# InterDigitalInc/VersatileFilmGrain

Hardware: AMD Instinct MI355X
Metric: Mpixels/s (Y+UV) + achieved HBM GB/s vs roofline, 4320p 10-bit 4:2:0 (higher is better)
Workload: dtype u16

## Files before the change

include/vfgs_hip.h:

```cpp
#ifndef VFGS_HIP_H
#define VFGS_HIP_H

#include <stdint.h>

#ifdef __cplusplus
extern "C" {
#endif

#define VFGS_HIP_MAX_PATTERNS 8


void vfgs_set_luma_pattern(int index, signed char* P);
void vfgs_set_chroma_pattern(int index, signed char* P);
void vfgs_set_scale_lut(int c, unsigned char lut[]);
void vfgs_set_pattern_lut(int c, unsigned char lut[]);
void vfgs_set_seed(unsigned int seed);
void vfgs_set_scale_shift(int shift);
void vfgs_set_depth(int depth);
void vfgs_set_legal_range(int legal);
void vfgs_set_chroma_subsampling(int subx, int suby);
void vfgs_add_grain_line(void* Y, void* U, void* V, int y, int width);


void vfgs_hip_line_lookahead(int enable);
// ... 87 lines not shown
int vfgs_hip_overlap_end(void* stream);

int vfgs_hip_init_devices(const int* devices, int n);

int vfgs_hip_supports_depth(int depth);

int vfgs_hip_dev_build(void);

int vfgs_hip_add_grain_frames_host(void* const* Y, void* const* U, void* const* V, unsigned nframes, unsigned width,
                                   unsigned height, unsigned stride, unsigned cstride);
void* vfgs_hip_host_alloc(uint64_t bytes);
void vfgs_hip_host_free(void* p);

int vfgs_hip_device_info(int* cu_count, int* lds_bytes_per_cu, int* clock_khz, char* name, int name_len);

typedef struct vfgs_hip_launch_info {
	int depth, csubx, csuby;
	int out8;
	int one_y, one_c;
	int in_place;
	int nframes;
	int workgroups_per_frame;
	int frames_per_front;
	int rows_per_wave[2];
	int positions_per_row[2];
	int parts_per_row;
	int persistent_luma_workgroups;
	int waves_per_workgroup;
	int lds_bytes_per_workgroup;
	unsigned long long launches;
	char kernel[96];
	int listed;
	int internal;
} vfgs_hip_launch_info;
int vfgs_hip_last_launch_info(vfgs_hip_launch_info* out);

#ifdef __cplusplus
}
#endif

#endif
```

versatilefilmgrain_amd/csrc/vfgs_fw_kernel.hip:

```cpp
#include <hip/hip_runtime.h>

#include "vfgs_fw_layout.h"
#include "vfgs_layout.h"

namespace vfgs {
namespace {

__device__ inline int noise_index(const uint32_t* w, int n)
{
	const uint64_t two = ((uint64_t)w[(n >> 5) + 1] << 32) | w[n >> 5];
	return (int)((two >> (n & 31)) & 2047u);
}

__device__ inline int clip127(int v) { return v > 127 ? 127 : (v < -127 ? -127 : v); }

__device__ inline void put_sample(const FwLaunch& L, const vfgs_hip_pattern_job& jb, int y, int x, int v)
{
	if (!jb.chroma)
		L.bank[(size_t)jb.index * 4096 + y * 64 + x] = (int8_t)v;
	else if (L.csubx == 2 && L.csuby == 2)
		L.bank[(size_t)(kSlots + jb.index) * 4096 + y * 64 + x] = (int8_t)v;
	else
		L.chroma_raw[jb.index * 1024 + y * 32 + x] = (int8_t)v;
}
// ... 231 lines not shown
	ImageLayout L;
	int one_y, one_c, slot_y, slot_cb, slot_cr;
	int pk16;
};

__global__ __launch_bounds__(256) void fw_patch_tables(const PatchArgs p)
{
	const int o = blockIdx.x * 256 + threadIdx.x;
	const ImageLayout& L = p.L;
	if (o < 64 * 64)
	{
		const int r = o >> 6, x = o & 63;
		uint8_t* dst = p.img + L.y_off + L.y_bank;
		if (p.one_y)
		{
			if (p.slot_y < kSlots && (p.mask_luma >> p.slot_y & 1))
			{
				const int v = p.bank[(size_t)p.slot_y * 4096 + o];
				if (p.pk16)
				{
					*(int16_t*)(dst + r * L.y_rs + 2 * x) = (int16_t)v;
					*(int16_t*)(dst + L.y_neg + r * L.y_rs + 2 * x) = (int16_t)-v;
				}
				else
				{
					dst[r * L.y_rs + x] = (uint8_t)v;
					dst[L.y_neg + r * L.y_rs + x] = (uint8_t)-v;
				}
			}
		}
		else
			for (int k = 0; k < kSlots; k++)
				if (p.mask_luma >> k & 1)
					dst[r * L.y_rs + x * kSlots + k] = (uint8_t)p.bank[(size_t)k * 4096 + o];
	}
	else if (o - 4096 < L.cw * L.ch)
	{
		const int q = o - 4096;
		const int r = q / L.cw, x = q % L.cw;
		if (p.one_c)
		{
			for (int c = 0; c < 2; c++)
			{
				const int k = c ? p.slot_cr : p.slot_cb;
				if (k < kSlots && (p.mask_chroma >> k & 1))
				{
					const int v = p.bank[(size_t)(kSlots + k) * 4096 + r * 64 + x];
					if (p.pk16)
					{
						*(int16_t*)(p.img + L.c_off[c] + L.c_bank + r * L.c_rs + 2 * x) = (int16_t)v;
						*(int16_t*)(p.img + L.c_off[c] + L.c_bank + L.c_neg + r * L.c_rs + 2 * x) = (int16_t)-v;
					}
					else
					{
						p.img[L.c_off[c] + L.c_bank + r * L.c_rs + x] = (uint8_t)v;
						p.img[L.c_off[c] + L.c_bank + L.c_neg + r * L.c_rs + x] = (uint8_t)-v;
					}
				}
			}
		}
		else
			for (int k = 0; k < kSlots; k++)
				if (p.mask_chroma >> k & 1)
					for (int c = 0; c < 2; c++)
						p.img[L.c_off[c] + L.c_bank + r * L.c_rs + x * kSlots + k] = (uint8_t)p.bank[(size_t)(kSlots + k) * 4096 + r * 64 + x];
	}
}

}

hipError_t launch_fw_generate(const FwLaunch& L, hipStream_t stream)
{
	bool ff = false, ar = false, chroma = false;
	for (int i = 0; i < L.njobs; i++)
	{
		(L.job[i].kind ? ar : ff) = true;
		chroma = chroma || L.job[i].chroma;
	}
	if (ff) hipLaunchKernelGGL(fw_ff_kernel, dim3(L.njobs), dim3(1024), 0, stream, L);
	if (ar) hipLaunchKernelGGL(fw_ar_kernel, dim3(L.njobs), dim3(256), 0, stream, L);
	if (chroma && !(L.csubx == 2 && L.csuby == 2))
		hipLaunchKernelGGL(fw_commit_chroma, dim3(L.njobs), dim3(256), 0, stream, L);
	return hipGetLastError();
}

hipError_t launch_fw_patch(uint8_t* img, const int8_t* bank, uint32_t mask_luma, uint32_t mask_chroma, int csubx, int csuby,
                           bool one_y, bool one_c, int slot_y, int slot_cb, int slot_cr, bool depth8, hipStream_t stream)
{
	PatchArgs p{};
	p.img = img; p.bank = bank; p.mask_luma = mask_luma; p.mask_chroma = mask_chroma;
	p.L = image_layout(csubx, csuby, one_y, one_c, depth8);
	p.pk16 = depth8 && kPk16;
	p.one_y = one_y; p.one_c = one_c; p.slot_y = slot_y; p.slot_cb = slot_cb; p.slot_cr = slot_cr;
	const int n = 4096 + p.L.cw * p.L.ch;
	hipLaunchKernelGGL(fw_patch_tables, dim3((n + 255) / 256), dim3(256), 0, stream, p);
	return hipGetLastError();
}

// ... 2 lines not shown
```

versatilefilmgrain_amd/csrc/vfgs_host.cpp:

```cpp
#include <hip/hip_runtime.h>

#include <sys/mman.h>
#include <unistd.h>

#include <algorithm>
#include <chrono>
#if defined(__SSE2__)
#include <emmintrin.h>
#endif
#include <cstdarg>
#include <cstdio>
#include <cstdlib>
#include <cstring>
#include <mutex>
#include <string>
#include <thread>
#include <vector>

#include "../../include/vfgs_hip.h"
#include "../../include/vfgs_hip_fw.h"
#include "vfgs_fw_layout.h"
#include "vfgs_layout.h"

namespace vfgs {
// ... 1006 lines not shown

int uniform_slot(const uint8_t (&plut)[256])
{
	const int k = plut[0] >> 4;
	for (int i = 1; i < 256; i++)
		if ((plut[i] >> 4) != k) return -1;
	return k;
}

void build_tables(const State& s, uint8_t* img, const vfgs::ImageLayout& L, bool one_y, bool one_c, const int (&slot)[3])
{
	memset(img, 0, L.bytes);
	const bool pk16 = s.bs == 0 && vfgs::kPk16;
	uint8_t* yb = img + L.y_off + L.y_bank;
	for (int r = 0; r < 64; r++)
		for (int x = 0; x < 64; x++)
		{
			if (one_y)
			{
				const int v = slot[0] < vfgs::kSlots ? s.bank[0][slot[0]][r][x] : 0;
				if (pk16)
				{
					const int16_t p = (int16_t)v, n = (int16_t)-v;
					memcpy(yb + r * L.y_rs + 2 * x, &p, 2);
					memcpy(yb + L.y_neg + r * L.y_rs + 2 * x, &n, 2);
				}
				else
				{
					yb[r * L.y_rs + x] = (uint8_t)v;
					yb[L.y_neg + r * L.y_rs + x] = (uint8_t)-v;
				}
			}
			else
				for (int k = 0; k < vfgs::kSlots; k++) yb[r * L.y_rs + x * vfgs::kSlots + k] = (uint8_t)s.bank[0][k][r][x];
		}
	for (int c = 0; c < 2; c++)
	{
		uint8_t* cb = img + L.c_off[c] + L.c_bank;
		for (int r = 0; r < L.ch; r++)
			for (int x = 0; x < L.cw; x++)
			{
				if (one_c)
				{
					const int v = slot[1 + c] < vfgs::kSlots ? s.bank[1][slot[1 + c]][r][x] : 0;
					if (pk16)
					{
						const int16_t p = (int16_t)v, n = (int16_t)-v;
						memcpy(cb + r * L.c_rs + 2 * x, &p, 2);
						memcpy(cb + L.c_neg + r * L.c_rs + 2 * x, &n, 2);
					}
					else
					{
						cb[r * L.c_rs + x] = (uint8_t)v;
						cb[L.c_neg + r * L.c_rs + x] = (uint8_t)-v;
					}
				}
				else
					for (int k = 0; k < vfgs::kSlots; k++) cb[r * L.c_rs + x * vfgs::kSlots + k] = (uint8_t)s.bank[1][k][r][x];
			}
	}
	for (int c = 0; c < 3; c++)
	{
		uint32_t* lut = (uint32_t*)(c == 0 ? img + L.y_off : img + L.c_off[c - 1] + L.c_lut[c - 1]);
		if (pk16 && (c == 0 ? one_y : one_c))
		{
			memcpy(lut, s.slut[c], 256);
			continue;
		}
		for (int i = 0; i < 256; i++)
		{
			const int sl = s.plut[c][i] >> 4;
			const uint32_t sel = sl < vfgs::kSlots ? (uint32_t)sl : 0x0cu;
			const int sc = s.slut[c][i] << (16 - s.scale_shift);
			lut[i] = (sel << 24) | ((uint32_t)sc & 0xffffffu);
			if (!(c == 0 ? one_y : one_c)) lut[256 + i] = (sel << 24) | ((uint32_t)(-sc) & 0xffffffu);
		}
	}
}

void digest_pluts(State& s)
{
	if (s.plut_seen) return;
	s.plut_bad_c = -1;
	for (int c = 0; c < 3; c++)
	{
		s.plut_slot[c] = uniform_slot(s.plut[c]);
		for (int i = 0; i < 256 && s.plut_bad_c < 0; i++)
			if ((s.plut[c][i] >> 4) > vfgs::kSlots) { s.plut_bad_c = c; s.plut_bad_i = i; }
	}
	s.plut_seen = true;
}
// ... 290 lines not shown
	}
	else
	{
		if (int e = upload_stream(s, lo, hi, stream)) return e;
		HIP_TRY(s.lfsr.use(stream));
		a.stream = s.lfsr.dev();
		a.stream_bytes = (uint32_t)(s.lfsr.dev_words() * 4);
		a.cur_bit0 = (uint32_t)(first_cur - s.lfsr.base_bit());
		a.up_bit0 = (uint32_t)(first_up - s.lfsr.base_bit());
		a.frame_bit_step = (uint32_t)frame_step;
	}

	const long per_frame = (long)a.pd[0].wgs + 2L * a.pd[1].wgs;
	if (per_frame > 0x3fffffffL || nframes > 65535) return fail(14, "launch too large");
	if (per_frame == 0) { if (seeds) seeded_done(); return 0; }
	bool persist = false;
	long grid = per_frame;
	if (VFGS_PERSIST_MIN_TASKS > 0 && s.bs != 0 && !wide && !s.img_one_y && a.pd[0].wgs > 0 &&
	    (size_t)vfgs::kWavesPerWG * a.pd[0].rw_rpw * a.pd[0].rowbytes <= ((size_t)VFGS_PERSIST_MAX_WG_KB << 10))
	{
		const long tasks = (long)a.pd[0].wgs * nframes, slots = (long)s.cu_count * 4;
		const long k = (tasks + slots - 1) / slots;
		if (k >= VFGS_PERSIST_MIN_TASKS)
		{
			const long P = (tasks + k - 1) / k;
			persist = true;
			a.persist_wgs = (int)P;
			a.persist_step_f = (int)(P / a.pd[0].wgs);
			a.persist_step_r = (int)(P % a.pd[0].wgs);
			grid = P + 2L * a.pd[1].wgs * nframes;
			if (grid > 0x7fffffffL) return fail(14, "launch too large");
		}
	}
#ifdef VFGS_NO_FRONTS
	a.lfronts = 0;
#else
	const bool in_region = g_states[0].ov.active && (stream == g_states[0].ov.s[0] || stream == g_states[0].ov.s[1]);
	a.lfronts = (!persist && nframes >= 2 && !in_region && 2 * (yext + 2 * cext) >= (64u << 20)) ? 1 : 0;
#endif
	if (mix)
	{
		if (!(s.img_one_y && s.img_one_c) || persist) return fail(19, "internal: the table image is not the form the chroma mix was admitted for");
		a.mix_kernel = 1;
		a.mix_lw = (int)width;
		for (int c = 0; c < 2; c++)
		{
			a.mix[c][0] = g_mix[c][0]; a.mix[c][1] = g_mix[c][1];
			a.mix[c][2] = g_mix[c][2] * (1 << s.bs);
			a.mix[c][3] = g_mix[c][3];
		}
		const uint64_t dext = dg.out8 ? (uint64_t)part_h * dg.stride : yext, dfp = dg.out8 ? dg.ypitch : ypitch;
		auto meet = [](uintptr_t p, uint64_t pn, uintptr_t q, uint64_t qn) { return p < q + qn && q < p + pn; };
		bool shared = false;
		if (!list)
			shared = meet((uintptr_t)sY, (uint64_t)(nframes - 1) * ypitch + yext, (uintptr_t)dY, (uint64_t)(nframes - 1) * dfp + dext);
		else
			for (unsigned i = 0; i < nframes && !shared; i++)
				for (unsigned j = 0; j < nframes && !shared; j++)
					shared = meet((uintptr_t)list->src[0][i], yext, (uintptr_t)list->dst[0][j], dext);
		if (shared)
		{
			a.mix_planes = 1;
			HIP_TRY(vfgs::launch_grain(a, list, 8 + s.bs, s.csubx, s.csuby, dg.out8, true, true, wide, false, (int)grid, stream));
			a.mix_planes = 2;
		}
	}
	HIP_TRY(vfgs::launch_grain(a, list, 8 + s.bs, s.csubx, s.csuby, dg.out8, s.img_one_y, s.img_one_c, wide, persist, (int)grid, stream));
	if (seeds) seeded_done();
	if (stripes && s.stripes.prepare_next(s.lfsr) != hipSuccess) (void)hipGetLastError();
	if (&s == &g_states[0])
	{
		vfgs_hip_launch_info& li = g_last_launch;
		const unsigned long long n = li.launches + 1;
		li = vfgs_hip_launch_info{};
		li.launches = n;
		li.depth = 8 + s.bs; li.csubx = s.csubx; li.csuby = s.csuby;
		li.out8 = dg.out8; li.one_y = s.img_one_y; li.one_c = s.img_one_c;
		li.in_place = (sY == dY && sU == dU && sV == dV);
		li.listed = a.listed;
		li.internal = g_internal_launch ? 1 : 0;
		li.nframes = (int)nframes;
		li.workgroups_per_frame = (int)per_frame;
		li.frames_per_front = 1 << a.lfronts;
		for (int pt = 0; pt < 2; pt++)
		{
			li.rows_per_wave[pt] = a.pd[pt].rw_rpw;
			li.positions_per_row[pt] = a.pd[pt].rw_segs;
		}
		li.parts_per_row = (int)nparts;
		li.persistent_luma_workgroups = persist ? a.persist_wgs : 0;
		li.waves_per_workgroup = vfgs::kWavesPerWG;
		const vfgs::ImageLayout L = vfgs::layout_of(s.csubx, s.csuby, s.img_one_y, s.img_one_c, s.bs == 0);
		li.lds_bytes_per_workgroup = vfgs::lds_allocation(s.bs != 0, s.img_one_y, s.img_one_c, wide, L.lds_bytes + vfgs::kParamBytes);
		vfgs::describe_launch(li.kernel, sizeof li.kernel, 8 + s.bs, s.csubx, s.csuby, dg.out8, s.img_one_y, s.img_one_c, wide, persist);
		if (mix)
		{
			li.lds_bytes_per_workgroup = vfgs::mix_lds_allocation(L.lds_bytes + vfgs::kParamBytes);
			snprintf(li.kernel, sizeof li.kernel, "grain_mix_kernel<%d,%d,%d,%s,%s>", 8 + s.bs, s.csubx, s.csuby, dg.out8 ? "true" : "false", wide ? "true" : "false");
			if (a.mix_planes) li.launches++;
		}
		g_last_launch_valid = true;
	}
	return 0;
}

int run_host(void* Y, void* U, void* V, unsigned y, unsigned width, unsigned height, unsigned stride, unsigned cstride, unsigned py, unsigned ph)
{
	State& s = S();
	if (int e = ensure_init(-1)) return e;
	if (height == 0) return 0;
	const unsigned sz = s.bs ? 2 : 1;
	const unsigned nblk = (width + 15) / 16;
	if (ph == 0)
	{
		if (int e = check_luts(s)) return e;
		advance_seeds(s, y, height, nblk, y);
		return 0;
	}
	const unsigned crow0 = py / s.csuby;
	const unsigned crows = (py + ph - 1) / s.csuby - crow0 + 1;
	const unsigned rows[3] = {ph, crows, crows};
	const unsigned rowlen[3] = {nblk * 16 * sz, nblk * 16 / s.csubx * sz, nblk * 16 / s.csubx * sz};
// ... 1374 lines not shown
```

versatilefilmgrain_amd/csrc/vfgs_kernel.hip:

```cpp
#include <hip/hip_runtime.h>
#include <stdint.h>
#include <stdio.h>

#include <type_traits>

#include "vfgs_layout.h"

namespace vfgs {

typedef uint32_t u32x4 __attribute__((ext_vector_type(4)));
typedef uint32_t u32x2 __attribute__((ext_vector_type(2)));
typedef uint32_t u32x3 __attribute__((ext_vector_type(3)));
typedef short s16x2 __attribute__((ext_vector_type(2)));
typedef unsigned short u16x2 __attribute__((ext_vector_type(2)));


__device__ __forceinline__ int pick_slot(uint32_t hi, uint32_t lo, uint32_t lut_entry)
{
	return (int)__builtin_amdgcn_perm(hi, lo, lut_entry) >> 24;
}

__device__ __forceinline__ int mad_i24(int x, uint32_t y, int c)
{
	int r;
// ... 60 lines not shown
constexpr uint32_t kOOB = 0x80000000u;

__device__ __forceinline__ __amdgpu_buffer_rsrc_t make_rsrc(const uint8_t* base, uint32_t bytes)
{
	return __builtin_amdgcn_make_buffer_rsrc((void*)base, 0, bytes, 0x00020000);
}

template <int NS, int BW>
struct LaneMap {
	static constexpr bool PAIR = (NS == 8 && BW == 16);
	static constexpr int SHIFT = PAIR ? 8 : BW / 2;
	static constexpr int NR = PAIR ? 1 : NS / BW + 1;
	static constexpr int NQ = NS / 4;
	static constexpr int NE = NR - 1;
	static constexpr int BPL = PAIR ? 1 : NS / BW;
	__device__ static constexpr int run(int q) { return PAIR ? 0 : (4 * q + BW - SHIFT) / BW; }
	__device__ static constexpr int col(int q) { return PAIR ? 4 * q : (4 * q + BW - SHIFT) % BW; }
	__device__ static constexpr int edge_quad(int e) { return PAIR ? 0 : ((e + 1) * BW - (BW - SHIFT)) / 4 - 1; }
};

template <int NR>
struct RunParam {
	uint32_t pa[NR];
};

template <int SUBX, int SUBY, int RS, int SB>
__device__ __forceinline__ uint32_t block_param(uint32_t v, uint32_t bank_off, int sx, int sy, int sb, bool* neg)
{
	const uint32_t fx = (v >> sx) & 0x3ff;
	const uint32_t fy = __builtin_amdgcn_alignbit(v, v, sy) & 0x3ff;
	const uint32_t ox = (__umul24(fx, 13u) >> 10) * (4 / SUBX);
	const uint32_t oy = (__umul24(fy, 12u) >> 10) * (4 / SUBY);
	*neg = (v >> sb) & 1;
	return __umul24(oy, (uint32_t)RS) + ox * SB + bank_off;
}

template <int DEPTH, int BW, bool OVERLAP, bool ONE, bool ALIGN2, int NEG, bool MIX = false>
__device__ __forceinline__ void grain_unit(const uint8_t* lds, uint32_t (&w)[4],
                                            const RunParam<LaneMap<DEPTH == 8 ? 16 : 8, BW>::NR>& rp,
                                            const RunParam<LaneMap<DEPTH == 8 ? 16 : 8, BW>::NR>& up,
                                            const uint32_t lutb, const uint32_t rowoff, const uint32_t uprowoff, const int wcur, const int wup,
                                            const bool (&edge_on)[LaneMap<DEPTH == 8 ? 16 : 8, BW>::PAIR ? 1 : LaneMap<DEPTH == 8 ? 16 : 8, BW>::NE],
                                            const bool first, const uint32_t lo2, const uint32_t hi2, const int pkshift, const uint32_t (&ix)[4])
{
	constexpr int NS = DEPTH == 8 ? 16 : 8;
	using M = LaneMap<NS, BW>;
	constexpr int NR = M::NR, NQ = M::NQ;
	auto index_dword = [&](int d) { return MIX ? ix[d] : w[d]; };
	constexpr bool PK = DEPTH == 8 && ONE && kPk16;
	static_assert(!(PK && M::PAIR), "lane pairs are 10-bit lanes");
	int sg[NR];
	uint32_t ad[NR], k2s[NR];
#pragma unroll
	for (int r = 0; r < NR; r++)
	{
		sg[r] = (int)rp.pa[r] >> 31;
		ad[r] = (rp.pa[r] & 0xffffu) + rowoff - ((ONE && OVERLAP) ? ((uint32_t)sg[r] & (uint32_t)NEG) : 0u);
		k2s[r] = ONE ? 0u : (OVERLAP ? lutb : (((uint32_t)sg[r] & 0x04000400u) | lutb));
	}
	if constexpr (PK && !OVERLAP)
	{
		const uint32_t rnd = 1u << (pkshift - 1);
		const uint32_t rpk = rnd * 0x10001u, shpk = (uint32_t)pkshift * 0x10001u;
		const uint8_t* lut = lds + (lutb & 0xffffu);
		uint32_t S[NS / 2], Pp[NS / 2], G[NS / 2];
#pragma unroll
		for (int q = 0; q < NQ; q++)
// ... 326 lines not shown
{
	constexpr int NS = DEPTH == 8 ? 16 : 8;
	constexpr int SZ = DEPTH > 8 ? 2 : 1;
	constexpr int SB = ONE ? ((DEPTH == 8 && kPk16) ? 2 : 1) : kSlots;
	using M = LaneMap<NS, BW>;
	constexpr int NR = M::NR;
	constexpr int RPB = 16 / SUBY;
	constexpr int NEF = M::PAIR ? 1 : M::NE;
	constexpr int K = M::SHIFT * SZ / 4;
	constexpr int DW = OUT8 ? 2 : 4;
	constexpr int KD = OUT8 ? K / 2 : K;
	static_assert(!OUT8 || (DEPTH > 8 && K % 2 == 0), "the narrowed destination exists for 16-bit containers");
	constexpr int LDA = VFGS_LDAUX_ALIGNED, STA = VFGS_STAUX_ALIGNED;
	constexpr int LPB = M::PAIR ? 1 : M::BPL;
	constexpr int BPS = M::PAIR ? 32 : 64 * M::BPL;
	constexpr int NU = MIX ? 2 : ((DEPTH > 8 && ONE && NARROW != 0) ? VFGS_RING_NARROW10 : ring_depth<DEPTH, ONE>());
	constexpr int GPP = kTileBlocks / (NU * BPS);
	static_assert(GPP * NU * BPS == kTileBlocks, "a part is a whole number of groups");
	constexpr uint32_t PT_CUR = IMG_BYTES, PT_UP = IMG_BYTES + kParamTableBytes;
	static_assert(IMG_BYTES % 16 == 0, "table image in whole 16-byte units");
	static_assert(!(PERSIST && (WIDE || NARROW != 0)), "persistent workgroups walk ordinary rows");
	static_assert(!MIX || (ONE && NARROW == 0 && !PERSIST), "the mix exists for one-pattern chroma walked row by row");
	const int pt = comp ? 1 : 0;
	auto uni = [](int v) { return __builtin_amdgcn_readfirstlane(v); };

	auto task = [&](const int f, const int r, const bool first_task) {
	const int split = r & (pd.rw_splits - 1);
	const int kbr = uni(r >> pd.rw_lsplits);
	const int Rabs = (a.y0 >> 4) + kbr;
	const int row_first = (a.y0 + SUBY - 1) / SUBY;
	const int prow0 = a.y0 / SUBY;
	const int alo = max(row_first, Rabs * RPB), ahi = min(row_first + pd.nrows, (Rabs + 1) * RPB);
	const int rpw = pd.rw_rpw;
#if VFGS_RW_CONSEC
	const int RSTR = 1;
	const int base = uni(Rabs * RPB + split * (kWavesPerWG * rpw) + wave * rpw);
	int k0 = max(0, alo - base), k1 = min(rpw, max(0, ahi - base));
#else
	constexpr int RSTR = kWavesPerWG;
	const int base = uni(Rabs * RPB + split * (kWavesPerWG * rpw) + wave);
	int k0 = (max(0, alo - base) + kWavesPerWG - 1) / kWavesPerWG, k1 = min(rpw, (max(0, ahi - base) + kWavesPerWG - 1) / kWavesPerWG);
#endif
	if (kbr >= a.nbrows || k1 < k0) k1 = k0;
	k0 = uni(k0); k1 = uni(k1);
	const bool wg_up = (Rabs > 0) && (split == 0);

	const int last = a.nblk - 1;
	const uint32_t cur_bit = a.cur_bit0 + (uint32_t)f * a.frame_bit_step + (uint32_t)(kbr * a.nblk);
	const uint32_t up_bit = (kbr > 0) ? cur_bit - (uint32_t)a.nblk : a.up_bit0 + (uint32_t)f * a.frame_bit_step;

	constexpr int STEP = kWavesPerWG * 64 * 16;
	constexpr int NIT = (IMG_BYTES + STEP - 1) / STEP;
	u32x4 tmp[NIT];
	if (!PERSIST || first_task)
	{
		const __amdgpu_buffer_rsrc_t irs = make_rsrc(a.tables + img_off, IMG_BYTES);
#pragma unroll
		for (int it = 0; it < NIT; it++)
			tmp[it] = __builtin_amdgcn_raw_buffer_load_b128(irs, min((uint32_t)(threadIdx.x * 16 + it * STEP), (uint32_t)(IMG_BYTES - 16)), 0, 0);
	}
	constexpr int NPE = (kParamEntries + kWavesPerWG * 64 - 1) / (kWavesPerWG * 64);
	const __amdgpu_buffer_rsrc_t strs = make_rsrc((const uint8_t*)a.stream, a.stream_bytes);
	const __amdgpu_buffer_rsrc_t strs_up = make_rsrc((const uint8_t*)a.stream, wg_up ? a.stream_bytes : 0);
	auto param_loads = [&](const int B0, u32x2 (&wc)[NPE], u32x2 (&wu)[NPE]) {
#pragma unroll
		for (int i = 0; i < NPE; i++)
		{
			const int e = (int)threadIdx.x + i * kWavesPerWG * 64;
			const uint32_t blk = (uint32_t)min(max(B0 + e - 1, 0), last);
			const bool need = e < a.nblk - B0 + 4 && e < kParamEntries;
			wc[i] = __builtin_amdgcn_raw_buffer_load_b64(strs, need ? ((cur_bit + blk) >> 5) * 4 : kOOB, 0, 0);
			wu[i] = __builtin_amdgcn_raw_buffer_load_b64(strs_up, need ? ((up_bit + blk) >> 5) * 4 : kOOB, 0, 0);
		}
	};
	const int fsx = comp == 0 ? 0 : (comp == 1 ? 10 : 20);
	const int fsy = comp == 0 ? 14 : (comp == 1 ? 24 : 4);
	const int fsb = comp == 0 ? 31 : (comp == 1 ? 2 : 15);
	auto param_table = [&](const int B0, const u32x2 (&wc)[NPE], const u32x2 (&wu)[NPE]) {
#pragma unroll
		for (int i = 0; i < NPE; i++)
		{
			if (i > 0 && i * kWavesPerWG * 64 >= a.nblk - B0 + 4) break;
			const int e = (int)threadIdx.x + i * kWavesPerWG * 64;
			const uint32_t blk = (uint32_t)min(max(B0 + e - 1, 0), last);
			bool neg;
			const uint32_t vc = __builtin_amdgcn_alignbit(wc[i].y, wc[i].x, (cur_bit + blk) & 31);
			const uint32_t pc = (block_param<SUBX, SUBY, RS, SB>(vc, bank_off, fsx, fsy, fsb, &neg) + ((ONE && neg) ? (uint32_t)NEG : 0u)) | (neg ? 0x80000000u : 0u);
			const uint32_t vu = __builtin_amdgcn_alignbit(wu[i].y, wu[i].x, (up_bit + blk) & 31);
			const uint32_t pu = block_param<SUBX, SUBY, RS, SB>(vu, bank_off, fsx, fsy, fsb, &neg) | (neg ? 0x80000000u : 0u);
			if (e < kParamEntries)
			{
				*(uint32_t*)(lds + PT_CUR + e * 4) = pc;
// ... 29 lines not shown
			lw[u][4 * i] = t.x; lw[u][4 * i + 1] = t.y; lw[u][4 * i + 2] = t.z; lw[u][4 * i + 3] = t.w;
		}
	};
	if constexpr (NARROW == 0)
	{
		const __amdgpu_buffer_rsrc_t rs0 = make_rsrc(sbase + (k0 < k1 ? row_off(k0) : 0u), k0 < k1 ? left(0) : 0u);
#pragma unroll
		for (int u = 0; u < NU; u++) load_seg<LDA>(rs0, lane16 + u * UB, 0, w[u]);
		if constexpr (MIX)
		{
#pragma unroll
			for (int u = 0; u < NU; u++)
			{
				const uint32_t o = (uint32_t)u * (UB * LQ);
				const bool on = k0 < k1 && o < pl.rowbytes;
				load_luma(make_rsrc(lbase + (on ? lrow_off(k0) + o : 0u), on ? min(pl.rowbytes - o, UB * LQ) : 0u), u);
			}
		}
	}
	else
	{
#pragma unroll
		for (int u = 0; u < NU; u++)
		{
			const int k = k0 + u / NARROW;
			const __amdgpu_buffer_rsrc_t rs0 = make_rsrc(sbase + (k < k1 ? row_off(k) : 0u), k < k1 ? pd.rowbytes : 0u);
			load_seg<LDA>(rs0, lane16 + (u % NARROW) * UB, 0, w[u]);
		}
	}
	if (!PERSIST || first_task)
	{
#pragma unroll
		for (int it = 0; it < NIT; it++)
			*(u32x4*)(lds + min((uint32_t)(threadIdx.x * 16 + it * STEP), (uint32_t)(IMG_BYTES - 16))) = tmp[it];
	}
	else
		__syncthreads();

	param_table(0, wc0, wu0);
	__syncthreads();
	const int nparts = WIDE ? (a.nblk + kTileBlocks - 1) / kTileBlocks : 1;
	static_assert(!(WIDE && NARROW != 0), "rows walked in parts are not narrow");
	if (k0 >= k1 && nparts == 1)
		return;

	const uint32_t lutb = lut_off * 0x10001u;
	const uint32_t lo2 = a.lo2[pt], hi2 = a.hi2[pt];
	const bool first = M::PAIR && (lane & 1);
	const uint32_t pairoff = M::PAIR ? (first ? 0u : 8u * SB) : 0u;
	const uint32_t idx0 = (M::PAIR ? (uint32_t)(lane + 1) >> 1 : (uint32_t)lane * LPB) * 4;
	const int cl = M::PAIR ? lane - 1 - (lane & 1) : lane * LPB - 1;
	constexpr int SSTEP = M::PAIR ? 64 : BPS;
	auto lane_up = [](uint32_t old, uint32_t v) { return (uint32_t)__builtin_amdgcn_update_dpp((int)old, (int)v, 0x138, 0xf, 0xf, false); };
	auto lane_down = [](uint32_t old, uint32_t v) { return (uint32_t)__builtin_amdgcn_update_dpp((int)old, (int)v, 0x130, 0xf, 0xf, false); };
	auto rot_up = [](uint32_t v) { return (uint32_t)__builtin_amdgcn_mov_dpp((int)v, 0x13c, 0xf, 0xf, false); };
	auto rot_down = [](uint32_t v) { return (uint32_t)__builtin_amdgcn_mov_dpp((int)v, 0x134, 0xf, 0xf, false); };
	auto results = [](const uint32_t (&t)[4], uint32_t (&o)[DW]) {
		if constexpr (OUT8)
		{
			uint32_t n[4];
#pragma unroll
			for (int d = 0; d < 4; d++) n[d] = ((t[d] + (0x00010001u << (DEPTH - 9))) >> (DEPTH - 8)) & 0x00ff00ffu;
			o[0] = __builtin_amdgcn_perm(n[1], n[0], 0x06040200);
			o[1] = __builtin_amdgcn_perm(n[3], n[2], 0x06040200);
		}
		else
		{
// ... 7 lines not shown
	const int mixc = comp == 2 ? 1 : 0;
	const int mix_lm = MIX ? a.mix[mixc][0] : 0, mix_cm = MIX ? a.mix[mixc][1] : 0, mix_off = MIX ? a.mix[mixc][2] : 0;
	const bool mix_on = MIX && a.mix[mixc][3] != 0;
	uint32_t outp[DW] = {};
	uint32_t tp[KD > 0 ? KD : 1] = {};
	__amdgpu_buffer_rsrc_t pdst = make_rsrc(dbase, 0);
	if constexpr (NARROW != 0)
	{
		constexpr int P = NARROW, RPG = NU / P;
		const int ngr = (k1 - k0 + RPG - 1) / RPG;
		for (int G = 0; G < ngr; G++)
		{
			const int kg = k0 + G * RPG;
#pragma unroll
			for (int u = 0; u < NU; u++)
			{
				const int p = u % P;
				const int k = kg + u / P;
				const bool valid = k < k1, nvalid = k + RPG < k1;
				const __amdgpu_buffer_rsrc_t nsrc = make_rsrc(sbase + (nvalid ? row_off(k + RPG) : 0u), nvalid ? pd.rowbytes : 0u);
				const __amdgpu_buffer_rsrc_t cdst = make_rsrc(dbase + (valid ? row_offd(k) : 0u), valid ? (OUT8 ? pd.drowbytes : pd.rowbytes) : 0u);
				uint32_t t[4];
#pragma unroll
				for (int d = 0; d < K; d++) t[d] = lane_up(p == 0 ? 0u : carry[d], w[u][4 - K + d]);
#pragma unroll
				for (int d = 0; d < K; d++) carry[d] = rot_up(w[u][4 - K + d]);
#pragma unroll
				for (int d = K; d < 4; d++) asm volatile("v_mov_b32 %0, %1" : "=v"(t[d]) : "v"(w[u][d - K]));
				load_seg<LDA>(nsrc, lane16 + p * UB, 0, w[u]);
				if (valid)
				{
					const int j = base + RSTR * k - Rabs * RPB;
					const int jrow = j * SUBY;
					const uint32_t rowoff = (uint32_t)j * RS, uprowoff = (uint32_t)(RPB + j) * RS;
					const int wc_ = jrow == 0 ? (SUBY > 1 ? 20 : 12) : 24, wu_ = jrow == 0 ? (SUBY > 1 ? 20 : 24) : 12;
					const uint8_t* pe = lds + idx0;
					bool edge_on[NEF];
					if (M::PAIR)
					{
						const int jl = cl + p * SSTEP;
						edge_on[0] = jl >= 0 && jl + 1 < 2 * a.nblk;
					}
					else
					{
#pragma unroll
						for (int ed = 0; ed < M::NE; ed++) edge_on[ed] = (cl + p * SSTEP + ed >= 0) && (cl + p * SSTEP + ed < last);
					}
					RunParam<NR> rp, up;
#pragma unroll
					for (int rr = 0; rr < NR; rr++) rp.pa[rr] = *(const uint32_t*)(pe + PT_CUR + (p * BPS + rr) * 4) + pairoff;
					if (Rabs > 0 && jrow <= 1)
					{
#pragma unroll
						for (int rr = 0; rr < NR; rr++) up.pa[rr] = *(const uint32_t*)(pe + PT_UP + (p * BPS + rr) * 4) + pairoff;
						grain_unit<DEPTH, BW, true, ONE, ONE && SUBX == 2, NEG>(lds, t, rp, up, lutb, rowoff, uprowoff, wc_, wu_, edge_on, first, lo2, hi2, a.pk_shift, t);
					}
					else
					{
#pragma unroll
						for (int rr = 0; rr < NR; rr++) up.pa[rr] = 0u;
						grain_unit<DEPTH, BW, false, ONE, ONE && SUBX == 2, NEG>(lds, t, rp, up, lutb, rowoff, uprowoff, 0, 0, edge_on, first, lo2, hi2, a.pk_shift, t);
					}
				}
				uint32_t o[DW];
				results(t, o);
#pragma unroll
				for (int d = 0; d < KD; d++) outp[DW - KD + d] = lane_down(rot_down(o[d]), tp[d]);
				store_unit<DW, STA>(pdst, laned + ((p + P - 1) % P) * UBD, outp);
				pdst = cdst;
#pragma unroll
				for (int d = KD; d < DW; d++) outp[d - KD] = o[d];
#pragma unroll
				for (int d = 0; d < KD; d++) tp[d] = o[d];
#if VFGS_SCHED_FENCE
				__builtin_amdgcn_sched_barrier(0);
#endif
			}
		}
#pragma unroll
		for (int d = 0; d < KD; d++) outp[DW - KD + d] = lane_down(0u, tp[d]);
		store_unit<DW, STA>(pdst, laned + (P - 1) * UBD, outp);
		return;
	}
	auto walk_row = [&](auto overlap, const int k, const int g_lo, const int g_hi) {
		constexpr bool OV = decltype(overlap)::value;
		const int j = base + RSTR * k - Rabs * RPB;
		const int jrow = j * SUBY;
		const uint32_t rowoff = (uint32_t)j * RS, uprowoff = (uint32_t)(RPB + j) * RS;
		const int wc_ = jrow == 0 ? (SUBY > 1 ? 20 : 12) : 24, wu_ = jrow == 0 ? (SUBY > 1 ? 20 : 24) : 12;
		const uint32_t ro = row_off(k), rod = row_offd(k);
		uint32_t lw1 = 0;
		const uint32_t lro = MIX ? lrow_off(k) : 0u;
		if constexpr (MIX && SUBX == 2)
		{
			const __amdgpu_buffer_rsrc_t lrs = make_rsrc(lbase + lro, pl.rowbytes);
			const uint32_t at = (uint32_t)(a.mix_lw - 1) * SZ;
			lw1 = SZ == 2 ? (uint32_t)(uint16_t)__builtin_amdgcn_raw_buffer_load_b16(lrs, at, 0, 0) : (uint32_t)(uint8_t)__builtin_amdgcn_raw_buffer_load_b8(lrs, at, 0, 0);
		}
		for (int g = g_lo; g < g_hi; g++)
		{
			const bool lastg = g + 1 == ngroups;
			const int ng = lastg ? 0 : g + 1;
			const bool nvalid = !lastg || k + 1 < k1;
			const uint32_t nso = nvalid ? (lastg ? row_off(k + 1) : ro) + (uint32_t)ng * GB : 0u;
			const __amdgpu_buffer_rsrc_t nsrc = make_rsrc(sbase + nso, nvalid ? left(ng) : 0u);
			const __amdgpu_buffer_rsrc_t cdst = make_rsrc(dbase + (rod + (uint32_t)g * GBD), leftd(g));
			const uint8_t* pe = lds + idx0 + (uint32_t)((g - g_lo) * NU * BPS * 4);
			const int clg = cl + g * NU * SSTEP;
#pragma unroll
			for (int u = 0; u < NU; u++)
			{
				const bool firsts = u == 0 && g == 0;
				uint32_t t[4];
				uint32_t ti[4] = {};
				if constexpr (MIX)
				{
					uint32_t mi[4];
					if (mix_on)
						mix_index<DEPTH, SUBX>(w[u], lw[u], mix_lm, mix_cm, mix_off, a.mix_lw - 1 - (((NU * g + u) * 64 + lane) * NS * SUBX), lw1, mi);
					else
					{
// ... 306 lines not shown
```

versatilefilmgrain_amd/csrc/vfgs_layout.h:

```cpp
#pragma once
#include <stdint.h>

namespace vfgs {

constexpr int kSlots = 8;
constexpr int kMaxUnits = 64;
constexpr int kBlock = 16;

#ifndef VFGS_WAVES
#define VFGS_WAVES 4
#endif
#ifndef VFGS_WG_PER_CU
#define VFGS_WG_PER_CU 4
#endif
#ifndef VFGS_SCHED_FENCE
#define VFGS_SCHED_FENCE 1
#endif
#ifndef VFGS_LDAUX_ALIGNED
#define VFGS_LDAUX_ALIGNED 2
#endif
#ifndef VFGS_STAUX_ALIGNED
#define VFGS_STAUX_ALIGNED 2
#endif
#ifndef VFGS_RING
#define VFGS_RING 4
#endif
#ifndef VFGS_RING_ONE10
#define VFGS_RING_ONE10 4
#endif
#ifndef VFGS_RING_PK
#define VFGS_RING_PK 2
#endif
#ifndef VFGS_RING_NARROW10
#define VFGS_RING_NARROW10 2
#endif
#ifndef VFGS_ONE10_WG_PER_CU
#define VFGS_ONE10_WG_PER_CU 4
#endif
#ifndef VFGS_ONE8_WG_PER_CU
#define VFGS_ONE8_WG_PER_CU 0
#endif
#ifndef VFGS_RW_CONSEC
#define VFGS_RW_CONSEC 0
#endif

#if !defined(VFGS_DEV_BUILD)
#if VFGS_WAVES != 4 || VFGS_WG_PER_CU != 4 || VFGS_RING != 4 || VFGS_RING_ONE10 != 4 || VFGS_RING_PK != 2 || VFGS_RING_NARROW10 != 2 || VFGS_ONE10_WG_PER_CU != 4 || VFGS_ONE8_WG_PER_CU != 0 || VFGS_SCHED_FENCE != 1 || VFGS_LDAUX_ALIGNED != 2 || VFGS_STAUX_ALIGNED != 2 || VFGS_RW_CONSEC != 0 || \
    defined(VFGS_NO_FRONTS) || defined(VFGS_NO_LOOKAHEAD) || defined(VFGS_NO_ONE_PATTERN) || defined(VFGS_NO_PK16) || defined(VFGS_PK_NO_READ2) || defined(VFGS_PK_WAVES) || defined(VFGS_ONE10_WAVES) ||  defined(VFGS_RW_WG_BYTES) || defined(VFGS_RW_MIN_FILL_PCT) || defined(VFGS_PERSIST_MIN_TASKS) || defined(VFGS_PERSIST_MAX_WG_KB)
#error "libvfgs_hip: a tuning knob differs from the shipped configuration; developer variants must define VFGS_DEV_BUILD"
#endif
#endif

constexpr int kWavesPerWG = VFGS_WAVES;
#ifdef VFGS_NO_PK16
constexpr bool kPk16 = false;
#else
constexpr bool kPk16 = true;
#endif

constexpr int kTileBlocks = 512;
constexpr int kParamEntries = kTileBlocks + 4;
constexpr int kParamTableBytes = (kParamEntries * 4 + 15) & ~15;
constexpr int kParamBytes = 2 * kParamTableBytes;

constexpr int kLdsPerCU = 163840;
constexpr int lds_allocation(const bool depth10, const bool one_y, const bool one_c, const bool wide, const int need)
{
	const int cap = (depth10 && one_y) ? VFGS_ONE10_WG_PER_CU : ((!depth10 && one_y && one_c && !wide) ? VFGS_ONE8_WG_PER_CU : 0);
	if (cap <= 0) return need;
	const int target = (kLdsPerCU / cap) & ~2047;
	const int next = (kLdsPerCU / (cap + 1)) & ~2047;
	return need > next ? need : (target < 65536 ? target : 65536);
}

constexpr int kMixWgPerCU = 4;
constexpr int mix_lds_allocation(const int need)
{
	const int target = (kLdsPerCU / kMixWgPerCU) & ~2047;
	return need > target ? need : target;
}

struct ImageLayout {
	int lut_bytes;
	int y_rs, c_rs;
	int y_bank, c_bank;
	int y_neg, c_neg;
	int y_bytes, c_bytes;
	int y_off, c_off[2];
	int c_lut[2];
	int bytes;
	int lds_bytes;
	int cw, ch;
};

constexpr ImageLayout image_layout(int csubx, int csuby, bool one_y, bool one_c, bool depth8)
{
	ImageLayout L{};
	L.lut_bytes = 2 * 256 * 4;
	L.cw = 64 / csubx;
	L.ch = 64 / csuby;
	depth8 = depth8 && kPk16;
	const int ob = depth8 ? 2 : 1;
	L.y_rs = one_y ? 64 * ob + 16 : 64 * kSlots + 16;
	L.c_rs = one_c ? L.cw * ob + 16 : L.cw * kSlots + 16;
	L.y_bank = one_y ? (depth8 ? 256 : L.lut_bytes / 2) : L.lut_bytes;
	L.c_bank = one_c ? (depth8 ? 256 : L.lut_bytes / 2) : L.lut_bytes;
	L.y_neg = one_y ? 64 * L.y_rs : 0;
	L.c_neg = one_c ? L.ch * L.c_rs : 0;
	L.y_bytes = L.y_bank + 64 * L.y_rs + L.y_neg;
	L.c_bytes = L.c_bank + L.ch * L.c_rs + L.c_neg;
	L.y_off = 0;
	L.c_off[0] = L.y_bytes;
	L.c_off[1] = L.y_bytes + L.c_bytes;
	L.c_lut[0] = 0;
	L.c_lut[1] = 0;
	L.bytes = L.y_bytes + 2 * L.c_bytes;
	L.lds_bytes = L.y_bytes > L.c_bytes ? L.y_bytes : L.c_bytes;
	return L;
}

struct PlaneDesc {
	uint32_t pitch, dpitch;
	uint64_t fpitch, dfpitch;
	uint32_t rowbytes, drowbytes;
	int nrows;
	int wgs;
	int rw_segs;
	int rw_rpw, rw_splits, rw_lsplits;
};

constexpr int kListFrames = 32;
struct FrameTable {
	const uint8_t* src[3][kListFrames];
	uint8_t* dst[3][kListFrames];
};

struct KernelArgs {
	const uint8_t* src[3];
	uint8_t* dst[3];
	PlaneDesc pd[2];
	const uint32_t* stream;
	uint32_t stream_bytes;
	const uint8_t* tables;
	uint32_t cur_bit0;
	uint32_t up_bit0;
	uint32_t frame_bit_step;
	int y0;
	int nblk;
	int nbrows;
	int nframes;
	int listed;
	int lfronts;
	int persist_wgs;
	int persist_step_f, persist_step_r;
	int pk_shift;
	uint32_t lo2[2], hi2[2];
	int mix_kernel;
	int mix_planes;
	int mix_lw;
	int mix[2][4];
};
// ... 3 lines not shown
```

versatilefilmgrain_amd/hw.py:

```python
from __future__ import annotations

import ctypes as C
import os
from pathlib import Path

from .build import LIB

_lib = None


class VfgsHipError(RuntimeError):
    pass


def _share_hip_runtime_with_torch() -> None:
    import importlib.util
    import sys
    if "torch" in sys.modules or os.environ.get("VFGS_HIP_NO_TORCH_RUNTIME"):
        return
    try:
        spec = importlib.util.find_spec("torch")
    except (ImportError, ValueError):
        return
    if spec is None or not spec.origin:
# ... 79 lines not shown
    lib.vfgs_hip_get_seeded_stream_stats.restype = None
    lib.vfgs_hip_get_seed_state.argtypes = [vp]
    lib.vfgs_hip_get_luts.argtypes = [i, vp, vp]
    lib.vfgs_hip_get_params.argtypes = [vp]
    lib.vfgs_hip_get_params.restype = None
    lib.vfgs_hip_last_error_string.restype = C.c_char_p
    lib.vfgs_hip_timer_begin.argtypes = [vp]
    lib.vfgs_hip_timer_end.argtypes = [vp, C.POINTER(C.c_float)]
    lib.vfgs_hip_device_info.argtypes = [C.POINTER(i), C.POINTER(i), C.POINTER(i), C.c_char_p, i]
    lib.vfgs_hip_line_lookahead.argtypes = [i]
    lib.vfgs_hip_line_lookahead.restype = None
    lib.vfgs_hip_declare_frame.argtypes = [vp, vp, vp, u, u, u, u]
    lib.vfgs_hip_add_grain_frames_host.argtypes = [C.POINTER(vp), C.POINTER(vp), C.POINTER(vp), u, u, u, u, u]
    lib.vfgs_hip_host_alloc.argtypes = [C.c_uint64]
    lib.vfgs_hip_host_alloc.restype = vp
    lib.vfgs_hip_host_free.argtypes = [vp]
    lib.vfgs_hip_host_free.restype = None
    lib.vfgs_hip_last_launch_info.argtypes = [C.POINTER(LaunchInfo)]
    lib.vfgs_hip_set_chroma_mix.argtypes = [i, i, i, i]
    lib.vfgs_hip_clear_chroma_mix.argtypes = []
    lib.vfgs_hip_clear_chroma_mix.restype = None
    lib.vfgs_hip_get_chroma_mix.argtypes = [i, C.POINTER(i)]
    lib.vfgs_hip_supports_depth.argtypes = [i]
    if lib.vfgs_hip_dev_build() and not os.environ.get("VFGS_ALLOW_DEV_BUILD"):
        raise VfgsHipError(f"{path} is a developer build (tuning / ablation knobs); set VFGS_ALLOW_DEV_BUILD=1 to load it anyway")
    _lib = lib
    return lib


class LaunchInfo(C.Structure):
    _fields_ = [("depth", C.c_int), ("csubx", C.c_int), ("csuby", C.c_int), ("out8", C.c_int), ("one_y", C.c_int), ("one_c", C.c_int),
                ("in_place", C.c_int), ("nframes", C.c_int), ("workgroups_per_frame", C.c_int), ("frames_per_front", C.c_int),
                ("rows_per_wave", C.c_int * 2), ("positions_per_row", C.c_int * 2), ("parts_per_row", C.c_int), ("persistent_luma_workgroups", C.c_int),
                ("waves_per_workgroup", C.c_int), ("lds_bytes_per_workgroup", C.c_int), ("launches", C.c_ulonglong), ("kernel", C.c_char * 96), ("listed", C.c_int), ("internal", C.c_int)]


class FramePtrs(C.Structure):
    _fields_ = [("Y", C.c_void_p), ("U", C.c_void_p), ("V", C.c_void_p)]


EXPORTS = [
    "vfgs_set_luma_pattern", "vfgs_set_chroma_pattern", "vfgs_set_scale_lut", "vfgs_set_pattern_lut",
    "vfgs_set_seed", "vfgs_set_scale_shift", "vfgs_set_depth", "vfgs_set_legal_range",
    "vfgs_set_chroma_subsampling", "vfgs_add_grain_line",
    "vfgs_add_grain_stripe", "vfgs_hip_init", "vfgs_hip_shutdown", "vfgs_hip_reset_state",
    "vfgs_hip_add_grain_stripe_dev", "vfgs_hip_add_grain_frame_dev", "vfgs_hip_add_grain_frame_part_dev",
    "vfgs_hip_add_grain_frames_dev", "vfgs_hip_add_grain_frames_part_dev", "vfgs_hip_add_grain_copy_dev",
    "vfgs_hip_add_grain_copy8_dev", "vfgs_hip_add_grain_frame_list_dev", "vfgs_hip_add_grain_frame_list_part_dev", "vfgs_hip_add_grain_frame_list_copy_dev",
    "vfgs_hip_add_grain_frame_list_copy8_dev", "vfgs_hip_get_seed_state", "vfgs_hip_get_luts", "vfgs_hip_get_params", "vfgs_hip_last_error",
    "vfgs_hip_last_error_string", "vfgs_hip_timer_begin", "vfgs_hip_timer_end", "vfgs_hip_device_info",
    "vfgs_hip_dev_build", "vfgs_hip_init_devices", "vfgs_hip_overlap_begin", "vfgs_hip_overlap_end", "vfgs_hip_get_stream_stats", "vfgs_hip_line_lookahead", "vfgs_hip_declare_frame",
    "vfgs_hip_get_stripe_stream_stats", "vfgs_hip_lfsr_segments",
    "vfgs_hip_add_grain_frame_list_seeded_dev", "vfgs_hip_add_grain_frame_list_seeded_part_dev", "vfgs_hip_add_grain_frame_list_seeded_copy_dev",
    "vfgs_hip_add_grain_frame_list_seeded_copy8_dev", "vfgs_hip_seed_segments", "vfgs_hip_get_seeded_stream_stats",
    "vfgs_hip_add_grain_frames_host", "vfgs_hip_host_alloc", "vfgs_hip_host_free", "vfgs_hip_last_launch_info",
    "vfgs_hip_set_chroma_mix", "vfgs_hip_clear_chroma_mix", "vfgs_hip_get_chroma_mix", "vfgs_hip_supports_depth",
]


def _b(data):
    return (C.c_char * len(data)).from_buffer_copy(bytes(data))


class VfgsHip:

    def __init__(self, device: int | None = None, reset: bool = True):
        self.lib = load()
# ... 156 lines not shown
    def host_alloc(self, nbytes):
        p = self.lib.vfgs_hip_host_alloc(nbytes)
        if not p:
            raise VfgsHipError(f"vfgs_hip_host_alloc({nbytes}): {self.lib.vfgs_hip_last_error_string().decode()}")
        return p

    def host_free(self, p):
        self.lib.vfgs_hip_host_free(p)

    def stream_stats(self):
        out = (C.c_uint64 * 4)()
        self.lib.vfgs_hip_get_stream_stats(out)
        return {"refills_in_stream": out[0], "windows_built_ahead": out[1], "switches_to_built_ahead": out[2], "window_words": out[3]}

    def stripe_stream_stats(self):
        out = (C.c_uint64 * 4)()
        self.lib.vfgs_hip_get_stripe_stream_stats(out)
        return {"built_in_stream": out[0], "built_ahead": out[1], "switches_to_built_ahead": out[2], "last_launch_used_it": bool(out[3])}

    def overlap_begin(self, stream=0):
        self._ck(self.lib.vfgs_hip_overlap_begin(stream))

    def overlap_end(self, stream=0):
        self._ck(self.lib.vfgs_hip_overlap_end(stream))

    def init_devices(self, devices):
        arr = (C.c_int * len(devices))(*devices)
        self._ck(self.lib.vfgs_hip_init_devices(arr, len(devices)))

    def last_launch_info(self):
        li = LaunchInfo()
        if self.lib.vfgs_hip_last_launch_info(C.byref(li)):
            return None
        d = {k: getattr(li, k) for k, _ in LaunchInfo._fields_ if k not in ("rows_per_wave", "positions_per_row", "kernel")}
        d["rows_per_wave"] = list(li.rows_per_wave)
        d["positions_per_row"] = list(li.positions_per_row)
        d["kernel"] = li.kernel.decode()
        return d

    def device_info(self):
        cu, lds, clk = C.c_int(), C.c_int(), C.c_int()
        name = C.create_string_buffer(128)
        self._ck(self.lib.vfgs_hip_device_info(C.byref(cu), C.byref(lds), C.byref(clk), name, 128))
        return {"cu_count": cu.value, "lds_per_cu": lds.value, "clock_khz": clk.value, "name": name.value.decode()}
```

Baseline: 959,900.

## Assign rows to workgroup splits by residue and stage only their bank window

Reorders the pattern bank rows in the staged image so that rows sharing a residue mod the group size are contiguous. Workgroup splits then take rows by residue and copy only their window of the bank into LDS instead of the whole image. The goal is less global-to-LDS staging traffic and fewer load/store iterations per workgroup. It adds row-offset remapping in the kernel and host packers, changes the halo condition for the upper row, and reports new launch-info fields. The remapping has to agree exactly between the bank packing and the kernel indexing.

```diff
diff --git a/include/vfgs_hip.h b/include/vfgs_hip.h
--- a/include/vfgs_hip.h
+++ b/include/vfgs_hip.h
@@ -143,6 +143,8 @@
 	char kernel[96];
 	int listed;
 	int internal;
+	int rows_by_residue[2];
+	int staged_image_bytes[2];
 } vfgs_hip_launch_info;
 int vfgs_hip_last_launch_info(vfgs_hip_launch_info* out);
 
diff --git a/versatilefilmgrain_amd/csrc/vfgs_fw_kernel.hip b/versatilefilmgrain_amd/csrc/vfgs_fw_kernel.hip
--- a/versatilefilmgrain_amd/csrc/vfgs_fw_kernel.hip
+++ b/versatilefilmgrain_amd/csrc/vfgs_fw_kernel.hip
@@ -287,7 +287,7 @@
 		else
 			for (int k = 0; k < kSlots; k++)
 				if (p.mask_luma >> k & 1)
-					dst[r * L.y_rs + x * kSlots + k] = (uint8_t)p.bank[(size_t)k * 4096 + o];
+					dst[bank_row_pos(r, 4) * L.y_rs + x * kSlots + k] = (uint8_t)p.bank[(size_t)k * 4096 + o];
 	}
 	else if (o - 4096 < L.cw * L.ch)
 	{
@@ -318,7 +318,7 @@
 			for (int k = 0; k < kSlots; k++)
 				if (p.mask_chroma >> k & 1)
 					for (int c = 0; c < 2; c++)
-						p.img[L.c_off[c] + L.c_bank + r * L.c_rs + x * kSlots + k] = (uint8_t)p.bank[(size_t)(kSlots + k) * 4096 + r * 64 + x];
+						p.img[L.c_off[c] + L.c_bank + bank_row_pos(r, L.ch / kBankGroupRows) * L.c_rs + x * kSlots + k] = (uint8_t)p.bank[(size_t)(kSlots + k) * 4096 + r * 64 + x];
 	}
 }
 
diff --git a/versatilefilmgrain_amd/csrc/vfgs_host.cpp b/versatilefilmgrain_amd/csrc/vfgs_host.cpp
--- a/versatilefilmgrain_amd/csrc/vfgs_host.cpp
+++ b/versatilefilmgrain_amd/csrc/vfgs_host.cpp
@@ -1062,7 +1062,7 @@
 				}
 			}
 			else
-				for (int k = 0; k < vfgs::kSlots; k++) yb[r * L.y_rs + x * vfgs::kSlots + k] = (uint8_t)s.bank[0][k][r][x];
+				for (int k = 0; k < vfgs::kSlots; k++) yb[vfgs::bank_row_pos(r, 4) * L.y_rs + x * vfgs::kSlots + k] = (uint8_t)s.bank[0][k][r][x];
 		}
 	for (int c = 0; c < 2; c++)
 	{
@@ -1086,7 +1086,7 @@
 					}
 				}
 				else
-					for (int k = 0; k < vfgs::kSlots; k++) cb[r * L.c_rs + x * vfgs::kSlots + k] = (uint8_t)s.bank[1][k][r][x];
+					for (int k = 0; k < vfgs::kSlots; k++) cb[vfgs::bank_row_pos(r, L.ch / vfgs::kBankGroupRows) * L.c_rs + x * vfgs::kSlots + k] = (uint8_t)s.bank[1][k][r][x];
 			}
 	}
 	for (int c = 0; c < 3; c++)
@@ -1443,6 +1443,8 @@
 			if (grid > 0x7fffffffL) return fail(14, "launch too large");
 		}
 	}
+	a.pd[0].rw_res = ((VFGS_RW_RES & 1) && !s.img_one_y && !persist && a.pd[0].rw_splits > 1) ? 1 : 0;
+	a.pd[1].rw_res = ((VFGS_RW_RES & 2) && !s.img_one_c && a.pd[1].rw_splits > 1) ? 1 : 0;
 #ifdef VFGS_NO_FRONTS
 	a.lfronts = 0;
 #else
@@ -1493,12 +1495,20 @@
 		li.nframes = (int)nframes;
 		li.workgroups_per_frame = (int)per_frame;
 		li.frames_per_front = 1 << a.lfronts;
+		const vfgs::ImageLayout Lq = vfgs::layout_of(s.csubx, s.csuby, s.img_one_y, s.img_one_c, s.bs == 0);
 		for (int pt = 0; pt < 2; pt++)
 		{
 			li.rows_per_wave[pt] = a.pd[pt].rw_rpw;
 			li.positions_per_row[pt] = a.pd[pt].rw_segs;
 		}
 		li.parts_per_row = (int)nparts;
+		for (int pt = 0; pt < 2; pt++)
+		{
+			const bool one = pt ? s.img_one_c : s.img_one_y;
+			const int G = pt ? 4 / (int)s.csuby : 4, bank = pt ? Lq.c_bank : Lq.y_bank, rs = pt ? Lq.c_rs : Lq.y_rs;
+			li.rows_by_residue[pt] = a.pd[pt].rw_res;
+			li.staged_image_bytes[pt] = a.pd[pt].rw_res && !one ? bank + vfgs::bank_window_rows(G, a.pd[pt].rw_splits) * rs : (pt ? Lq.c_bytes : Lq.y_bytes);
+		}
 		li.persistent_luma_workgroups = persist ? a.persist_wgs : 0;
 		li.waves_per_workgroup = vfgs::kWavesPerWG;
 		const vfgs::ImageLayout L = vfgs::layout_of(s.csubx, s.csuby, s.img_one_y, s.img_one_c, s.bs == 0);
diff --git a/versatilefilmgrain_amd/csrc/vfgs_kernel.hip b/versatilefilmgrain_amd/csrc/vfgs_kernel.hip
--- a/versatilefilmgrain_amd/csrc/vfgs_kernel.hip
+++ b/versatilefilmgrain_amd/csrc/vfgs_kernel.hip
@@ -116,7 +116,15 @@
 	const uint32_t ox = (__umul24(fx, 13u) >> 10) * (4 / SUBX);
 	const uint32_t oy = (__umul24(fy, 12u) >> 10) * (4 / SUBY);
 	*neg = (v >> sb) & 1;
+	if constexpr (SB == kSlots) return __umul24(__umul24(fy, 12u) >> 10, (uint32_t)RS) + ox * SB + bank_off;
 	return __umul24(oy, (uint32_t)RS) + ox * SB + bank_off;
+}
+
+template <int SUBY, int RS, bool ONE>
+__device__ __forceinline__ uint32_t bank_rowoff(const int j, const int wfirst)
+{
+	if constexpr (ONE) return (uint32_t)j * RS;
+	else return (uint32_t)(bank_row_pos(j, 4 / SUBY) - wfirst) * RS;
 }
 
 template <int DEPTH, int BW, bool OVERLAP, bool ONE, bool ALIGN2, int NEG, bool MIX = false>
@@ -509,18 +517,27 @@
 	const int prow0 = a.y0 / SUBY;
 	const int alo = max(row_first, Rabs * RPB), ahi = min(row_first + pd.nrows, (Rabs + 1) * RPB);
 	const int rpw = pd.rw_rpw;
+	constexpr bool RESK = !ONE && !PERSIST && !VFGS_RW_CONSEC;
+	const bool res = RESK && pd.rw_res != 0;
+	const int lres = res ? pd.rw_lsplits : 0;
 #if VFGS_RW_CONSEC
 	const int RSTR = 1;
 	const int base = uni(Rabs * RPB + split * (kWavesPerWG * rpw) + wave * rpw);
 	int k0 = max(0, alo - base), k1 = min(rpw, max(0, ahi - base));
 #else
-	constexpr int RSTR = kWavesPerWG;
-	const int base = uni(Rabs * RPB + split * (kWavesPerWG * rpw) + wave);
-	int k0 = (max(0, alo - base) + kWavesPerWG - 1) / kWavesPerWG, k1 = min(rpw, (max(0, ahi - base) + kWavesPerWG - 1) / kWavesPerWG);
+	const int RSTR = RESK ? kWavesPerWG << lres : kWavesPerWG;
+	const int base = uni(Rabs * RPB + (res ? split + (wave << lres) : split * (kWavesPerWG * rpw) + wave));
+	constexpr int LW = kWavesPerWG == 1 ? 0 : (kWavesPerWG == 2 ? 1 : (kWavesPerWG == 4 ? 2 : (kWavesPerWG == 8 ? 3 : 4)));
+	static_assert((1 << LW) == kWavesPerWG, "waves per workgroup: a power of two");
+	int k0 = (max(0, alo - base) + RSTR - 1) >> (LW + lres), k1 = min(rpw, (max(0, ahi - base) + RSTR - 1) >> (LW + lres));
 #endif
 	if (kbr >= a.nbrows || k1 < k0) k1 = k0;
 	k0 = uni(k0); k1 = uni(k1);
-	const bool wg_up = (Rabs > 0) && (split == 0);
+	const bool wg_up = (Rabs > 0) && (split == 0 || (res && SUBY == 1 && split == 1));
+	constexpr int GRP = 4 / SUBY;
+	const int wfirst = res ? (pd.rw_splits == 4 ? bank_group(split, 4) : split) * ((GRP * kBankGroupRows) >> lres) : 0;
+	const uint32_t wskip = (uint32_t)wfirst * RS;
+	const uint32_t stage_bytes = res ? bank_off + (uint32_t)((GRP * kBankGroupRows) >> lres) * RS : (uint32_t)IMG_BYTES;
 
 	const int last = a.nblk - 1;
 	const uint32_t cur_bit = a.cur_bit0 + (uint32_t)f * a.frame_bit_step + (uint32_t)(kbr * a.nblk);
@@ -534,7 +551,11 @@
 		const __amdgpu_buffer_rsrc_t irs = make_rsrc(a.tables + img_off, IMG_BYTES);
 #pragma unroll
 		for (int it = 0; it < NIT; it++)
-			tmp[it] = __builtin_amdgcn_raw_buffer_load_b128(irs, min((uint32_t)(threadIdx.x * 16 + it * STEP), (uint32_t)(IMG_BYTES - 16)), 0, 0);
+		{
+			if (RESK && (uint32_t)(it * STEP) >= stage_bytes) break;
+			const uint32_t d = min((uint32_t)(threadIdx.x * 16 + it * STEP), stage_bytes - 16);
+			tmp[it] = __builtin_amdgcn_raw_buffer_load_b128(irs, (RESK && d >= bank_off) ? d + wskip : d, 0, 0);
+		}
 	}
 	constexpr int NPE = (kParamEntries + kWavesPerWG * 64 - 1) / (kWavesPerWG * 64);
 	const __amdgpu_buffer_rsrc_t strs = make_rsrc((const uint8_t*)a.stream, a.stream_bytes);
@@ -630,7 +651,10 @@
 	{
 #pragma unroll
 		for (int it = 0; it < NIT; it++)
-			*(u32x4*)(lds + min((uint32_t)(threadIdx.x * 16 + it * STEP), (uint32_t)(IMG_BYTES - 16))) = tmp[it];
+		{
+			if (RESK && (uint32_t)(it * STEP) >= stage_bytes) break;
+			*(u32x4*)(lds + min((uint32_t)(threadIdx.x * 16 + it * STEP), stage_bytes - 16)) = tmp[it];
+		}
 	}
 	else
 		__syncthreads();
@@ -704,7 +728,7 @@
 				{
 					const int j = base + RSTR * k - Rabs * RPB;
 					const int jrow = j * SUBY;
-					const uint32_t rowoff = (uint32_t)j * RS, uprowoff = (uint32_t)(RPB + j) * RS;
+					const uint32_t rowoff = bank_rowoff<SUBY, RS, ONE>(j, wfirst), uprowoff = bank_rowoff<SUBY, RS, ONE>(RPB + j, wfirst);
 					const int wc_ = jrow == 0 ? (SUBY > 1 ? 20 : 12) : 24, wu_ = jrow == 0 ? (SUBY > 1 ? 20 : 24) : 12;
 					const uint8_t* pe = lds + idx0;
 					bool edge_on[NEF];
@@ -758,7 +782,7 @@
 		constexpr bool OV = decltype(overlap)::value;
 		const int j = base + RSTR * k - Rabs * RPB;
 		const int jrow = j * SUBY;
-		const uint32_t rowoff = (uint32_t)j * RS, uprowoff = (uint32_t)(RPB + j) * RS;
+		const uint32_t rowoff = bank_rowoff<SUBY, RS, ONE>(j, wfirst), uprowoff = bank_rowoff<SUBY, RS, ONE>(RPB + j, wfirst);
 		const int wc_ = jrow == 0 ? (SUBY > 1 ? 20 : 12) : 24, wu_ = jrow == 0 ? (SUBY > 1 ? 20 : 24) : 12;
 		const uint32_t ro = row_off(k), rod = row_offd(k);
 		uint32_t lw1 = 0;
diff --git a/versatilefilmgrain_amd/csrc/vfgs_layout.h b/versatilefilmgrain_amd/csrc/vfgs_layout.h
--- a/versatilefilmgrain_amd/csrc/vfgs_layout.h
+++ b/versatilefilmgrain_amd/csrc/vfgs_layout.h
@@ -43,9 +43,12 @@
 #ifndef VFGS_RW_CONSEC
 #define VFGS_RW_CONSEC 0
 #endif
+#ifndef VFGS_RW_RES
+#define VFGS_RW_RES 3
+#endif
 
 #if !defined(VFGS_DEV_BUILD)
-#if VFGS_WAVES != 4 || VFGS_WG_PER_CU != 4 || VFGS_RING != 4 || VFGS_RING_ONE10 != 4 || VFGS_RING_PK != 2 || VFGS_RING_NARROW10 != 2 || VFGS_ONE10_WG_PER_CU != 4 || VFGS_ONE8_WG_PER_CU != 0 || VFGS_SCHED_FENCE != 1 || VFGS_LDAUX_ALIGNED != 2 || VFGS_STAUX_ALIGNED != 2 || VFGS_RW_CONSEC != 0 || \
+#if VFGS_WAVES != 4 || VFGS_WG_PER_CU != 4 || VFGS_RING != 4 || VFGS_RING_ONE10 != 4 || VFGS_RING_PK != 2 || VFGS_RING_NARROW10 != 2 || VFGS_ONE10_WG_PER_CU != 4 || VFGS_ONE8_WG_PER_CU != 0 || VFGS_SCHED_FENCE != 1 || VFGS_LDAUX_ALIGNED != 2 || VFGS_STAUX_ALIGNED != 2 || VFGS_RW_CONSEC != 0 || VFGS_RW_RES != 3 || \
     defined(VFGS_NO_FRONTS) || defined(VFGS_NO_LOOKAHEAD) || defined(VFGS_NO_ONE_PATTERN) || defined(VFGS_NO_PK16) || defined(VFGS_PK_NO_READ2) || defined(VFGS_PK_WAVES) || defined(VFGS_ONE10_WAVES) ||  defined(VFGS_RW_WG_BYTES) || defined(VFGS_RW_MIN_FILL_PCT) || defined(VFGS_PERSIST_MIN_TASKS) || defined(VFGS_PERSIST_MAX_WG_KB)
 #error "libvfgs_hip: a tuning knob differs from the shipped configuration; developer variants must define VFGS_DEV_BUILD"
 #endif
@@ -79,6 +82,12 @@
 	const int target = (kLdsPerCU / kMixWgPerCU) & ~2047;
 	return need > target ? need : target;
 }
+
+constexpr int kBankGroupRows = 16;
+constexpr int bank_group(int res, int G) { return G == 4 ? (((res & 1) << 1) | (res >> 1)) : res; }
+constexpr int bank_row_pos(int rho, int G) { return bank_group(rho & (G - 1), G) * kBankGroupRows + rho / G; }
+constexpr int bank_window_rows(int G, int R) { return G * kBankGroupRows / R; }
+constexpr int bank_window_first(int split, int G, int R) { return (R == 4 ? bank_group(split, 4) : split) * bank_window_rows(G, R); }
 
 struct ImageLayout {
 	int lut_bytes;
@@ -127,6 +136,7 @@
 	int wgs;
 	int rw_segs;
 	int rw_rpw, rw_splits, rw_lsplits;
+	int rw_res;
 };
 
 constexpr int kListFrames = 32;
diff --git a/versatilefilmgrain_amd/hw.py b/versatilefilmgrain_amd/hw.py
--- a/versatilefilmgrain_amd/hw.py
+++ b/versatilefilmgrain_amd/hw.py
@@ -135,7 +135,8 @@
     _fields_ = [("depth", C.c_int), ("csubx", C.c_int), ("csuby", C.c_int), ("out8", C.c_int), ("one_y", C.c_int), ("one_c", C.c_int),
                 ("in_place", C.c_int), ("nframes", C.c_int), ("workgroups_per_frame", C.c_int), ("frames_per_front", C.c_int),
                 ("rows_per_wave", C.c_int * 2), ("positions_per_row", C.c_int * 2), ("parts_per_row", C.c_int), ("persistent_luma_workgroups", C.c_int),
-                ("waves_per_workgroup", C.c_int), ("lds_bytes_per_workgroup", C.c_int), ("launches", C.c_ulonglong), ("kernel", C.c_char * 96), ("listed", C.c_int), ("internal", C.c_int)]
+                ("waves_per_workgroup", C.c_int), ("lds_bytes_per_workgroup", C.c_int), ("launches", C.c_ulonglong), ("kernel", C.c_char * 96), ("listed", C.c_int), ("internal", C.c_int),
+                ("rows_by_residue", C.c_int * 2), ("staged_image_bytes", C.c_int * 2)]
 
 
 class FramePtrs(C.Structure):
@@ -358,9 +359,10 @@
         li = LaunchInfo()
         if self.lib.vfgs_hip_last_launch_info(C.byref(li)):
             return None
-        d = {k: getattr(li, k) for k, _ in LaunchInfo._fields_ if k not in ("rows_per_wave", "positions_per_row", "kernel")}
-        d["rows_per_wave"] = list(li.rows_per_wave)
-        d["positions_per_row"] = list(li.positions_per_row)
+        pairs = ("rows_per_wave", "positions_per_row", "rows_by_residue", "staged_image_bytes")
+        d = {k: getattr(li, k) for k, _ in LaunchInfo._fields_ if k not in pairs + ("kernel",)}
+        for k in pairs:
+            d[k] = list(getattr(li, k))
         d["kernel"] = li.kernel.decode()
         return d
 
```

Result: no change. 965,900, median of 6 (+0.6%).
